# nellogrb/MultigridAnisotropicDiffusion

Hardware: AMD Instinct MI355X
Metric: Mvoxel-smooths/s (and V-cycles/s) at 512^3 fp32; achieved HBM GB/s vs peak (higher is better)
Workload: dtype f32

## Files before the change

### multigridanisotropicdiffusion_amd/build.py

```python
import os
import shutil
import subprocess
import sys

HERE = os.path.dirname(os.path.abspath(__file__))
CSRC = os.path.join(HERE, "csrc")
OUT = os.path.join(HERE, "libmad_hip.so")
SOURCES = ["mad_solver.hip"]
DEPS = ["../../include/mad.h", "../../include/mad_ved.h", "../../include/mad_ced.h",
        "../../include/mad_pm.h"]


def deps():
    return [f for f in os.listdir(CSRC) if f.endswith((".hip", ".hpp"))] + DEPS


def hipcc():
    for cand in (os.environ.get("HIPCC"), "/opt/rocm/bin/hipcc", shutil.which("hipcc")):
        if cand and os.path.exists(cand):
            return cand
    raise RuntimeError("hipcc not found")


def up_to_date():
    if not os.path.exists(OUT):
        return False
    t = os.path.getmtime(OUT)
    return all(os.path.getmtime(os.path.join(CSRC, d)) <= t for d in deps())


def build(force=False, verbose=True):
    if not force and up_to_date():
        return OUT
    cmd = [hipcc(), "--offload-arch=gfx950", "-O3", "-std=c++17", "-fPIC", "-shared",
           "-Wall", "-Wno-unused-function", "-o", OUT + ".tmp"]
    cmd += [os.path.join(CSRC, s) for s in SOURCES]
    cmd += ["-lrccl", "-lrocsolver", "-lrocblas"]
    if verbose:
        print(" ".join(cmd), flush=True)
    subprocess.check_call(cmd, cwd=HERE)
    os.replace(OUT + ".tmp", OUT)
    return OUT


if __name__ == "__main__":
    build(force="--force" in sys.argv)
```

### multigridanisotropicdiffusion_amd/csrc/mad_kernels.hpp

```cpp
#pragma once
#include <hip/hip_runtime.h>

#include <climits>
#include <type_traits>
#include <cstdint>

namespace mad {

enum { KISO = 1, KDIAG = 2, KFULL = 3 };

template <int DIM, int KIND>
struct CoefLayout {
  static constexpr int NA = (KIND == KISO) ? 1 : DIM;
  static constexpr int NG = DIM;
  static constexpr int NE = (KIND == KFULL) ? DIM * (DIM - 1) / 2 : 0;
  static constexpr int N = NA + NG + NE;
};

inline int coef_count(int dim, int kind) {
  int na = (kind == KISO) ? 1 : dim;
  int ne = (kind == KFULL) ? dim * (dim - 1) / 2 : 0;
  return na + dim + ne;
}

// ... 810 lines not shown
template <typename T, int DIM, int KIND>
__global__ void __launch_bounds__(256) residual_k(const T* __restrict__ u, const T* __restrict__ b,
                                                  T* __restrict__ r, const T* __restrict__ cf,
                                                  Geo g, Rat<T> rat, double* __restrict__ part) {
  const int k = (DIM == 3) ? (int)blockIdx.z : 0;
  const int j = blockIdx.y * blockDim.y + threadIdx.y;
  const int i = blockIdx.x * blockDim.x + threadIdx.x;
  double sq = 0.0;
  if (i < g.nx && j < g.ny) {
    const int64_t p = i + g.sy * j + g.sz * k;
    T D, S;
    stencil_terms<T, DIM, KIND>(u, cf, g, rat, i, j, k, p, D, S);
    const T rv = resid_value(b[p], D, u[p], S);
    r[p] = rv;
    sq = (double)rv * (double)rv;
  }
  if (part) {
    const double s = block_sum<256>(sq);
    if (threadIdx.x == 0 && threadIdx.y == 0)
      part[blockIdx.x + gridDim.x * (blockIdx.y + gridDim.y * blockIdx.z)] = s;
  }
}

template <typename T, int KIND, int TX, int TY, bool BREC = false, typename TE = T, typename TB = T>
__global__ void __launch_bounds__(TX * TY) resid3_k(const T* __restrict__ u, const TB* __restrict__ b,
                                                    T* __restrict__ r, const T* __restrict__ cf,
                                                    Geo g, Rat<T> rat, int zc, int ntx,
                                                    double* __restrict__ part,
                                                    TE* __restrict__ be = nullptr,
                                                    TE* __restrict__ xe = nullptr,
                                                    const TE* __restrict__ ue = nullptr,
                                                    T* __restrict__ uo = nullptr,
                                                    TE* __restrict__ bse = nullptr) {
  constexpr int NT = TX * TY;
  constexpr int RX = TX + 2, RY = TY + 2, PL = RX * RY;
  constexpr int UPT = (PL + NT - 1) / NT;
  constexpr int NCF = CoefLayout<3, KIND>::N;
  constexpr int RS = NCF + (BREC ? 1 : 0);
  constexpr uint32_t TS = sizeof(T);
  __shared__ T ring[4 * PL];
  const int tiles_per_plane = ntx * ((g.ny + TY - 1) / TY);
  const int chunk = blockIdx.x / tiles_per_plane;
  const int tile = blockIdx.x - chunk * tiles_per_plane;
  const int tyi = tile / ntx, txi = tile - (tile / ntx) * ntx;
  const int x0 = txi * TX, y0 = tyi * TY;
  const int tid = threadIdx.x;
  const int tx = tid % TX, ty = tid / TX;
// ... 5 lines not shown
  int u_dst[UPT];
  uint32_t u_src[UPT];
#pragma unroll
  for (int e = 0; e < UPT; ++e) {
    const int q = tid + e * NT;
    const int lj = q / RX, li = q - (q / RX) * RX;
    u_dst[e] = q < PL ? q : -1;
    u_src[e] = (uint32_t)(mirror(y0 - 1 + lj, ny) * sy + mirror(x0 - 1 + li, nx)) * TS;
  }
  const int i = x0 + tx, j = y0 + ty;
  const bool ok = i < nx && j < ny;
  const uint32_t rec_off = ok ? (uint32_t)(ty * sy + (tx & 1) * hx0 + (tx >> 1)) * (TS * RS) : 0u;
  const uint32_t pt_off = ok ? (uint32_t)(ty * sy + tx) * TS : 0u;
  const uint32_t pt_off_b = ok ? (uint32_t)(ty * sy + tx) * (uint32_t)sizeof(TB) : 0u;
  const int64_t rbase = (int64_t)y0 * sy + (x0 >> 1), pbase = (int64_t)y0 * sy + x0;
  const int il = (ty + 1) * RX + (tx + 1);
  constexpr int oyp = RX, oym = -RX;

  T up[UPT];
  T raw[RS];
  T bv = T(0);
  auto load_plane = [&](int m) {
    m = min(max(m, zlo), zhi - 1);
    const __amdgpu_buffer_rsrc_t rs = buf_rsrc(u + (int64_t)m * sz);
#pragma unroll
    for (int e = 0; e < UPT; ++e) up[e] = buf_load<T>(rs, u_src[e], 0u);
    if (ue) {
      const __amdgpu_buffer_rsrc_t re = buf_rsrc(ue + (int64_t)m * sz);
#pragma unroll
      for (int e = 0; e < UPT; ++e)
        up[e] = up[e] + (T)buf_load<TE>(re, (u_src[e] / TS) * (uint32_t)sizeof(TE), 0u);
    }
  };
  auto put_plane = [&](int m) {
    T* P = ring + (m & 3) * PL;
#pragma unroll
    for (int e = 0; e < UPT; ++e)
      if (e < UPT - 1 || u_dst[e] >= 0) P[u_dst[e]] = up[e];
  };
  auto load_pt = [&](int m) {
    m = min(max(m, 0), g.nz - 1);
    buf_load_rec<T, RS>(buf_rsrc(cf + ((int64_t)m * sz + rbase) * RS), rec_off, raw);
    if constexpr (!BREC) bv = (T)buf_load<TB>(buf_rsrc(b + (int64_t)m * sz + pbase), pt_off_b, 0u);
  };

  if (z0 - 1 >= zlo) {
// ... 627 lines not shown
            vz = fma(wy[bq], fma(wx[x][1], row[ix[x][1]], wx[x][0] * row[ix[x][0]]), vz);
          }
          v = fma(wz[c], vz, v);
        }
        out.v[x] = ADD ? xc[q].v[x] + v : v;
      }
      if (ok) *reinterpret_cast<V*>(fine + pxy + gf.sz * (int64_t)kk) = out;
    }
    __syncthreads();
#pragma unroll
    for (int q = 0; q < G; ++q) xc[q] = xn[q];
  }
}

template <typename T>
__global__ void __launch_bounds__(256) bsplit_k(const T* __restrict__ b, T* __restrict__ bs, Geo g, int p0) {
  const int k = p0 + (int)blockIdx.z;
  const int j = blockIdx.y * blockDim.y + threadIdx.y;
  const int i = blockIdx.x * blockDim.x + threadIdx.x;
  if (i >= g.nx || j >= g.ny) return;
  bs[cidx(g, i, j, k)] = b[i + g.sy * j + g.sz * (int64_t)k];
}

template <typename T>
__global__ void __launch_bounds__(256) brec_scatter_k(const T* __restrict__ b, T* __restrict__ cf,
                                                      Geo g, int ncf, int p0) {
  const int k = p0 + (int)blockIdx.z;
  const int j = blockIdx.y * blockDim.y + threadIdx.y;
  const int i = blockIdx.x * blockDim.x + threadIdx.x;
  if (i >= g.nx || j >= g.ny) return;
  cf[cidx(g, i, j, k) * g.rs + ncf] = b[i + g.sy * j + g.sz * (int64_t)k];
}

template <typename T>
__device__ __forceinline__ double coarse_row_dot(const double* __restrict__ a, const T* __restrict__ b,
                                                 int n, int lane) {
  double s = 0.0;
  for (int c = lane; c < n; c += 64) s += a[c] * (double)b[c];
  return wave_sum(s);
}

template <typename T>
__global__ void __launch_bounds__(256) coarse_solve_k(const double* __restrict__ inv,
                                                      const T* __restrict__ b, T* __restrict__ x,
                                                      int n) {
  const int row = blockIdx.x * 4 + (threadIdx.x >> 6);
// ... 356 lines not shown
```

### multigridanisotropicdiffusion_amd/csrc/mad_solver.hip

```cpp
#include <hip/hip_runtime.h>
#include <rocblas/rocblas.h>
#include <rocsolver/rocsolver.h>

#include <algorithm>
#include <chrono>
#include <cmath>
#include <cstdio>
#include <cstdlib>
#include <cstring>
#include <memory>
#include <mutex>
#include <stdexcept>
#include <string>
#include <thread>
#include <type_traits>
#include <vector>

#include "../../include/mad.h"
#include "mad_alloc.hpp"
#include "mad_coarse.hpp"
#include "mad_comm.hpp"
#include "mad_kernels.hpp"

using namespace mad;
// ... 852 lines not shown

  ZRange part_range(LevelData<T>& L, int tiles, const FusedCfg& fc, int part, int* flip,
                    uint32_t** sig) {
    const int nz = L.g.nz;
    ZRange zr = whole_range(nz, tiles, fc);
    *flip = (c_->d.gs_kernel == 4 && part == 0) ? 1 : 0;
    *sig = nullptr;
    if (part == 3 || part == 4) {
      REQUIRE(zr.nchunks >= 2 && zr.zc >= GHOST, MAD_ERR_UNSUPPORTED, "slab too thin for the single-launch sweep");
      *flip = 1;
      *sig = part == 3 ? L.sig : nullptr;
    } else if (part == 1) {
      zr = ZRange{0, boundary_planes(), nz - boundary_planes(), 2};
    } else if (part == 2) {
      const int ni = nz - 2 * boundary_planes();
      int chunks = std::max(1, std::min((fc.blocks + tiles - 1) / tiles, std::max(1, ni / 16)));
      const int zc = (ni + chunks - 1) / chunks;
      zr = ZRange{boundary_planes(), zc, zc, (ni + zc - 1) / zc};
    }
    return zr;
  }

  template <int KD, int TX, int TY, int NT>
  void launch_fused(LevelData<T>& L, const FusedCfg& fc, int part, bool zu = false) {
    const int ntx = (L.g.nx + TX - 1) / TX, nty = (L.g.ny + TY - 1) / TY;
    const int tiles = ntx * nty;
    int flip = 0;
    uint32_t* sig = nullptr;
    const ZRange zr = part_range(L, tiles, fc, part, &flip, &sig);
    const unsigned nb = (unsigned)(tiles * zr.nchunks);
    constexpr int NC = (KD == KFULL) ? 4 : 2;
    using FG = FusedGeom<NC, TX, TY>;
    constexpr size_t lds_u = sizeof(T) * FG::NP * FG::PLANE;
    REQUIRE(lds_u <= 160 * 1024, MAD_ERR_UNSUPPORTED,
            "fused GS tile needs " + std::to_string(lds_u) + " B of LDS (> 160 KiB)");
    constexpr size_t lds_bl = sizeof(T) * (FG::NP + NC) * FG::PLANE;
    constexpr bool bl_fits = lds_bl <= 160 * 1024;
    const bool bl = fused_b_lds(L);
    const size_t lds = bl ? lds_bl : lds_u;
    constexpr int MW = sizeof(T) == 8 ? 2 : 4;
    const PeerOut<T> po = part == 4 ? peer_out(L, buffer_index(L, L.t)) : PeerOut<T>{{nullptr, nullptr}, {nullptr, nullptr}};
    auto run = [&](auto kern) {
      {
        static std::mutex attr_mu;
        static std::vector<const void*> attr;
        std::lock_guard<std::mutex> lk(attr_mu);
        if (std::find(attr.begin(), attr.end(), (const void*)kern) == attr.end()) {
          HIP_CHECK(hipFuncSetAttribute((const void*)kern, hipFuncAttributeMaxDynamicSharedMemorySize,
                                        (int)lds));
          attr.push_back((const void*)kern);
        }
      }
      hipLaunchKernelGGL(kern, dim3(nb), dim3(NT), lds, c_->stream, L.x, L.t, L.bs ? L.bs : L.b, L.cf, L.g,
                         L.rat, zr.zc, ntx, nty, zr.zbase, zr.zstride, flip, sig, po);
    };
    if (part == 4) {
      if (L.brec)
        run(gs_fused3_k<T, KD, TX, TY, NT, MW, 2, true, true>);
      else if constexpr (bl_fits) {
        if (L.bs)
          run(gs_fused3_k<T, KD, TX, TY, NT, MW, 2, false, true, false, false, true>);
        else
          bl ? run(gs_fused3_k<T, KD, TX, TY, NT, MW, 2, false, true, true>)
             : run(gs_fused3_k<T, KD, TX, TY, NT, MW, 2, false, true>);
      } else
        run(gs_fused3_k<T, KD, TX, TY, NT, MW, 2, false, true>);
    } else if (L.brec) {
      run(gs_fused3_k<T, KD, TX, TY, NT, MW, 2, true>);
    } else if constexpr (bl_fits) {
      if (zu) {
        REQUIRE(part == 0, MAD_ERR_STATE, "zero-iterate sweep on a rank slab");
        if (L.bs)
          run(gs_fused3_k<T, KD, TX, TY, NT, MW, 2, false, false, false, true, true>);
        else
          bl ? run(gs_fused3_k<T, KD, TX, TY, NT, MW, 2, false, false, true, true>)
             : run(gs_fused3_k<T, KD, TX, TY, NT, MW, 2, false, false, false, true>);
      } else if (L.bs) {
        run(gs_fused3_k<T, KD, TX, TY, NT, MW, 2, false, false, false, false, true>);
// ... 4 lines not shown
    } else {
      REQUIRE(!zu, MAD_ERR_STATE, "zero-iterate sweep without its instance");
      run(gs_fused3_k<T, KD, TX, TY, NT, MW, 2>);
    }
  }

#ifndef MAD_FUSED_B_LDS
#define MAD_FUSED_B_LDS 1
#endif
  bool fused_b_lds(const LevelData<T>& L) const {
    return MAD_FUSED_B_LDS && sizeof(T) == 4 && !L.brec && !L.bs && &L == &lv_[0];
  }

#ifndef MAD_FUSED_F32_TY
#define MAD_FUSED_F32_TY 32
#endif
  void fused_shape(const LevelData<T>& L, int* tiles, int* nchunks) const {
    const FusedCfg fc = fused_cfg();
    const int tx = 64, ty = (c_->kind == KFULL && sizeof(T) == 4) ? MAD_FUSED_F32_TY : 16;
    *tiles = ((L.g.nx + tx - 1) / tx) * ((L.g.ny + ty - 1) / ty);
    *nchunks = whole_range(L.g.nz, *tiles, fc).nchunks;
  }

  void launch_fused_part(LevelData<T>& L, int part, bool zu = false) {
    const FusedCfg fc = fused_cfg();
    if (c_->kind == KFULL) {
      if constexpr (sizeof(T) == 4)
        launch_fused<KFULL, 64, MAD_FUSED_F32_TY, MAD_FUSED_F32_TY * 32>(L, fc, part, zu);
      else
        launch_fused<KFULL, 64, 16, 512>(L, fc, part, zu);
    } else if (c_->kind == KDIAG) {
      launch_fused<KDIAG, 64, 16, 1024>(L, fc, part, zu);
    } else {
      launch_fused<KISO, 64, 16, 1024>(L, fc, part, zu);
    }
    HIP_CHECK(hipGetLastError());
  }

  std::string smooth_kernel(int l) override {
    (void)l;
    const char* tn = sizeof(T) == 4 ? "float" : "double";
    const int dim = c_->dim, kind = c_->kind;
    char buf[160];
    if (c_->d.smoother == MAD_WEIGHTED_JACOBI) {
      const LevelData<T>& L = lv_[l];
      if (dim == 3 && L.g.nx >= 16 && L.g.ny >= 16)
        std::snprintf(buf, sizeof buf, "wj3_k<%s, %d, 64, 16, %s>", tn, kind, L.brec ? "true" : "false");
      else
        std::snprintf(buf, sizeof buf, "wj_k<%s, %d, %d>", tn, dim, kind);
    } else if (c_->d.smoother == MAD_GAUSS_SEIDEL_LEX) {
      std::snprintf(buf, sizeof buf, "gs_lex_plane_k<%s, %d, %d>", tn, dim, kind);
    } else if (!use_fused(l)) {
      std::snprintf(buf, sizeof buf, "gs_color_k<%s, %d, %d>", tn, dim, kind);
      if (lv_[l].peer) return std::string(buf) + " [rank slab: peer halo, edge planes pushed after the last colour pass]";
    } else {
      const int tx = 64, ty = (kind == KFULL && sizeof(T) == 4) ? MAD_FUSED_F32_TY : 16;
      const int nt = (kind == KFULL && sizeof(T) == 8) ? 512 : (kind == KFULL ? MAD_FUSED_F32_TY * 32 : 1024);
// ... 75 lines not shown
      std::swap(L.x, L.t);
      std::swap(L.alloc[0], L.alloc[3]);
      L.x_halo_ok = true;
      L.x_peer_pending = true;
      return 0.f;
    }
    const bool overlap = sweep_overlap(l);
    int tiles = 0, nchunks = 0;
    if (overlap) fused_shape(L, &tiles, &nchunks);
    if (overlap && L.sig && nchunks >= 2) {
      launch_fused_part(L, 3);
      wait_all_pending();
      const uint32_t target = ++L.sig_epoch * (uint32_t)tiles;
      if (L.g.zlo_ghost)
        HIP_CHECK(hipStreamWaitValue32(c_->comm_stream, L.sig, target, hipStreamWaitValueGte, 0xFFFFFFFFu));
      if (L.g.zhi_ghost)
        HIP_CHECK(hipStreamWaitValue32(c_->comm_stream, L.sig + 1, target, hipStreamWaitValueGte,
                                       0xFFFFFFFFu));
      c_->comm.exchange_planes(L.t, L.g.sz, L.g.nz, GHOST, L.g.zlo_ghost, L.g.zhi_ghost, sizeof(T),
                               std::is_same<T, double>::value, c_->comm_stream);
      HIP_CHECK(hipEventRecord(L.ev_halo, c_->comm_stream));
    } else if (!overlap) {
      const bool zu = (zero_x0_ && &L == &lv_[0]) || L.x_zero_lazy;
      zero_x0_ = false;
      L.x_zero_lazy = false;
      launch_fused_part(L, 0, zu);
    } else {
      launch_fused_part(L, 1);
      wait_all_pending();
      HIP_CHECK(hipEventRecord(L.ev_bnd, c_->stream));
      HIP_CHECK(hipStreamWaitEvent(c_->comm_stream, L.ev_bnd, 0));
      c_->comm.exchange_planes(L.t, L.g.sz, L.g.nz, GHOST, L.g.zlo_ghost, L.g.zhi_ghost, sizeof(T),
                               std::is_same<T, double>::value, c_->comm_stream);
      HIP_CHECK(hipEventRecord(L.ev_halo, c_->comm_stream));
      launch_fused_part(L, 2);
    }
    if (e1) HIP_CHECK(hipEventRecord(e1, c_->stream));
    std::swap(L.x, L.t);
    std::swap(L.alloc[0], L.alloc[3]);
    if (overlap) {
      L.x_halo_ok = true;
      L.x_halo_pending = true;
    } else {
      L.x_halo_ok = false;
    }
    return 0.f;
  }

  void prep_wj(int l) {
// ... 98 lines not shown
  }

  double finish_norm2(int64_t nparts, bool global) {
    hipLaunchKernelGGL(reduce_final_k, dim3(1), dim3(256), 0, c_->stream, part_, nparts, scal_);
    HIP_CHECK(hipGetLastError());
    if (global && c_->comm.active()) {
      wait_all_pending();
      c_->comm.allreduce_sum_f64(scal_, 1, c_->stream);
    }
    HIP_CHECK(hipMemcpyAsync(hscal_, scal_, sizeof(double), hipMemcpyDeviceToHost, c_->stream));
    HIP_CHECK(hipStreamSynchronize(c_->stream));
    return hscal_[0];
  }

  double residual(int l, bool want_norm) override { return residual_impl(l, want_norm, true); }

  bool refine_emitted_ = false;
  bool refine_emitted_bs_ = false;
  bool refine_fold_ok() const {
    const LevelData<T>& L = lv_[0];
    return c_->dim == 3 && L.g.nx >= 16 && L.g.ny >= 16 && !c_->geom[0].distributed;
  }
  bool zero_x0_ = false;
  bool lazy_zero_ok(int l) const {
#ifdef MAD_NO_LAZY_ZERO
    return false;
#else
    const auto& d = c_->d;
    return sizeof(T) == 4 && l >= 1 && l < c_->nlev - 1 && !c_->comm.active() && !d.verbose &&
           d.iterations_per_grid >= 1 && use_fused(l) && d.gs_kernel != 4 && !lv_[l].brec &&
           c_->dim == 3;
#endif
  }
  bool zero_sweep_ok() const {
#ifdef MAD_NO_ZERO_SWEEP
    return false;
#else
    const auto& d = c_->d;
    return sizeof(T) == 4 && refine_fold_ok() && !c_->comm.active() && d.cycle == MAD_VCYCLE &&
           !d.verbose && d.iterations_per_grid >= 1 && c_->nlev > 1 && use_fused(0) && d.gs_kernel != 4 &&
           !lv_[0].brec;
#endif
  }
  double residual64(bool fold = false) {
    LevelData<T>& L = lv_[0];
    if (fold && !refine_fold_ok()) {
      hipLaunchKernelGGL((add_conv_k<T>), dim3(flat_blocks(L.g.N)), dim3(256), 0, c_->stream, u64_, L.x, L.g.N);
      HIP_CHECK(hipGetLastError());
      fold = false;
    }
    if (c_->comm.active() && c_->geom[0].distributed) {
      wait_all_pending();
      c_->comm.exchange_planes(u64_, L.g.sz, L.g.nz, 1, L.g.zlo_ghost, L.g.zhi_ghost, sizeof(double),
                               true, c_->stream);
    }
    Geo g = L.g;
    g.rs = ncoef_;
    int64_t nparts = 0;
    if (c_->dim == 3 && g.nx >= 16 && g.ny >= 16) {
      constexpr int TX = 64, TY = 16;
      const int ntx = (g.nx + TX - 1) / TX, nty = (g.ny + TY - 1) / TY;
      int chunks = std::max(1, std::min((1024 + ntx * nty - 1) / (ntx * nty), g.nz / 8));
      const int zc = (g.nz + chunks - 1) / chunks;
      chunks = (g.nz + zc - 1) / zc;
      nparts = (int64_t)ntx * nty * chunks;
      REQUIRE(nparts <= part_cap_, MAD_ERR_UNSUPPORTED, "residual partials buffer too small");
      T* const bse = (L.bs && !c_->geom[0].distributed) ? L.bs : nullptr;
      refine_emitted_bs_ = bse != nullptr;
      auto go = [&](auto K) {
        constexpr int KD = decltype(K)::value;
        auto launch = [&](auto bptr) {
          using TB = std::remove_const_t<std::remove_pointer_t<decltype(bptr)>>;
          if (fold)
            hipLaunchKernelGGL((resid3_k<double, KD, TX, TY, false, T, TB>), dim3((unsigned)nparts),
                               dim3(TX * TY), 0, c_->stream, u64_, bptr, (double*)nullptr, cf64_, g, rat64_, zc,
                               ntx, part_, L.b, (T*)nullptr, (const T*)L.x, r64_, bse);
          else
            hipLaunchKernelGGL((resid3_k<double, KD, TX, TY, false, T, TB>), dim3((unsigned)nparts),
                               dim3(TX * TY), 0, c_->stream, u64_, bptr, (double*)nullptr, cf64_, g, rat64_, zc,
                               ntx, part_, L.b, L.x, (const T*)nullptr, (double*)nullptr, bse);
        };
#ifdef MAD_NO_B32_RHS
        launch((const double*)b64_);
#else
        if (b32_exact_)
          launch((const float*)b32_);
        else
          launch((const double*)b64_);
#endif
      };
      refine_emitted_ = true;
      if (c_->kind == KFULL) go(std::integral_constant<int, KFULL>{});
      else if (c_->kind == KDIAG) go(std::integral_constant<int, KDIAG>{});
      else go(std::integral_constant<int, KISO>{});
      if (fold) {
        std::swap(u64_, r64_);
        if (!zero_sweep_ok())
          hipLaunchKernelGGL((fill_k<T>), dim3(flat_blocks(L.g.N)), dim3(256), 0, c_->stream, L.x, L.g.N, T(0));
      }
    } else {
      dim3 gr = grid_for(g.nx, g.ny, g.nz, BLK);
      nparts = (int64_t)gr.x * gr.y * gr.z;
      REQUIRE(nparts <= part_cap_, MAD_ERR_UNSUPPORTED, "residual partials buffer too small");
      dispatch(c_->dim, c_->kind, [&](auto D, auto K) {
        hipLaunchKernelGGL((residual_k<double, D.value, K.value>), gr, BLK, 0, c_->stream, u64_, b64_,
                           r64_, cf64_, g, rat64_, part_);
      });
      refine_emitted_ = refine_emitted_bs_ = false;
    }
    HIP_CHECK(hipGetLastError());
    return std::sqrt(finish_norm2(nparts, c_->geom[0].distributed));
  }

  double norm64(const double* a) {
    const int64_t n = lv_[0].g.N;
    unsigned nb = flat_blocks(n, 2048);
    hipLaunchKernelGGL((sumsq_k<double>), dim3(nb), dim3(256), 0, c_->stream, a, n, part_);
    HIP_CHECK(hipGetLastError());
// ... 279 lines not shown
      lv_[0].x_halo_ok = false;
    if (!lv_[0].brec && !lv_[0].b_halo_ok) {
      halo(0, lv_[0].b, GHOST);
      lv_[0].b_halo_ok = true;
    }
    wait_all_pending();
    for (size_t l = 1; l < lv_.size(); ++l) {
      lv_[l].x_halo_ok = false;
      lv_[l].b_halo_ok = lv_[l].brec_ok = false;
    }
  }

  void vcycle_fast() {
    const bool ranks = c_->comm.active();
    if (c_->d.verbose || c_->bench_trace() || vgraph_failed_ || (ranks && !vgraph_ranks_ok()) ||
        (ranks && vcycles_eager_ < 1)) {
      if (ranks) ++vcycles_eager_;
      vcycle_rec(0);
      return;
    }
    sync_brec(0);
    sync_bsplit(0);
    if (ranks) ranks_graph_entry();
    const bool zu = zero_x0_;
    if (vgraph_) {
      bool same = vgraph_ptrs_.size() == lv_.size() && vgraph_zu_ == zu;
      for (size_t l = 0; same && l < lv_.size(); ++l)
        same = vgraph_ptrs_[l].first == lv_[l].x && vgraph_ptrs_[l].second == lv_[l].t &&
               vgraph_seq_[l] == (lv_[l].peer_seq & 1);
      if (!same) {
        HIP_CHECK(hipStreamSynchronize(c_->stream));
        (void)hipGraphExecDestroy(vgraph_);
        vgraph_ = nullptr;
      }
    }
    if (!vgraph_) {
      struct Snap {
        T* x;
        T* t;
        T* a0;
        T* a3;
        bool bh;
        int seq;
      };
      auto snap = [&] {
        std::vector<Snap> v;
        for (auto& L : lv_) v.push_back({L.x, L.t, L.alloc[0], L.alloc[3], L.b_halo_ok, L.peer_seq});
        return v;
      };
      auto restore = [&](const std::vector<Snap>& v) {
        for (size_t l = 0; l < lv_.size(); ++l) {
          lv_[l].x = v[l].x;
          lv_[l].t = v[l].t;
          lv_[l].alloc[0] = v[l].a0;
          lv_[l].alloc[3] = v[l].a3;
          lv_[l].b_halo_ok = v[l].bh;
          lv_[l].peer_seq = v[l].seq;
        }
      };
// ... 5 lines not shown
      try {
        vcycle_rec(0);
        if (ranks) {
          wait_all_pending();
          peer_resolve_all();
        }
      } catch (...) {
        (void)hipStreamEndCapture(c_->stream, &gph);
        if (gph) (void)hipGraphDestroy(gph);
        gph = nullptr;
        restore(before);
        if (!ranks) throw;
        captured = false;
      }
      if (captured && hipStreamEndCapture(c_->stream, &gph) != hipSuccess) {
        gph = nullptr;
        captured = false;
      }
      const std::vector<Snap> after = snap();
      bool same = captured;
      for (size_t l = 0; same && l < before.size(); ++l)
        same = before[l].x == after[l].x && before[l].t == after[l].t &&
               ((before[l].seq ^ after[l].seq) & 1) == 0;
      vgraph_exit_flags_ = halo_flags();
      restore(before);
      if (ranks) {
        for (size_t l = 0; l < lv_.size(); ++l) {
          lv_[l].x_halo_ok = flags_before[l].x_ok;
          lv_[l].b_halo_ok = flags_before[l].b_ok;
          lv_[l].brec_ok = flags_before[l].brec_ok;
          lv_[l].x_halo_pending = false;
        }
      }
      if (same && hipGraphInstantiate(&vgraph_, gph, nullptr, nullptr, 0) != hipSuccess) {
        vgraph_ = nullptr;
        same = false;
      }
      if (gph) (void)hipGraphDestroy(gph);
      zero_x0_ = zu;
      if (!same) {
        (void)hipGetLastError();
        vgraph_failed_ = true;
        vcycle_rec(0);
        return;
      }
      vgraph_zu_ = zu;
      zero_x0_ = false;
      vgraph_ptrs_.clear();
      vgraph_seq_.clear();
      for (auto& L : lv_) {
        vgraph_ptrs_.emplace_back(L.x, L.t);
        vgraph_seq_.push_back(L.peer_seq & 1);
      }
    }
    HIP_CHECK(hipGraphLaunch(vgraph_, c_->stream));
    zero_x0_ = false;
    if (ranks) c_->comm.graph_launched(c_->stream);
    if (ranks) {
      for (size_t l = 0; l < lv_.size(); ++l) {
        lv_[l].x_halo_ok = vgraph_exit_flags_[l].x_ok;
        lv_[l].b_halo_ok = vgraph_exit_flags_[l].b_ok;
        lv_[l].brec_ok = vgraph_exit_flags_[l].brec_ok;
        lv_[l].x_halo_pending = false;
      }
    } else {
      for (size_t l = 1; l < lv_.size(); ++l) lv_[l].b_halo_ok = lv_[l].brec_ok = false;
    }
  }

  void vcycle() override { vcycle_fast(); }

  void fmg() override { fmg_rec(0); }

  void per_sweep_line(int l, int it, const char* what, bool bench) {
    if (!c_->d.verbose) {
      const double rn = residual(l, true);
      c_->trace_push(c_->trace_rhs > 0.0 ? rn / c_->trace_rhs : rn);
      return;
    }
    const double rel = verbose_line(l, it, what);
    if (bench) {
      const double rn = rel * norm(l, MAD_B);
      c_->trace_push(c_->trace_rhs > 0.0 ? rn / c_->trace_rhs : rn);
    }
  }
// ... 29 lines not shown
    }
    if (refine_) {
      convert_to(src, in_dtype, b64_, N, c_->stream);
      b32_exact_ = in_dtype == MAD_U8 || in_dtype == MAD_I8 || in_dtype == MAD_U16 || in_dtype == MAD_I16 ||
                   in_dtype == MAD_F32;
      if (b32_exact_) {
        hipLaunchKernelGGL((convert_k<double, float>), dim3(nb), dim3(256), 0, c_->stream, b64_, b32_, N);
        HIP_CHECK(hipGetLastError());
      }
    } else {
      convert_in(src, in_dtype, L0.b, N);
      L0.b_halo_ok = L0.brec_ok = false;
    }
    auto to_fp32_rhs = [&](const double* a) {
      hipLaunchKernelGGL((convert_k<double, T>), dim3(nb), dim3(256), 0, c_->stream, a, L0.b, N);
      HIP_CHECK(hipGetLastError());
      L0.b_halo_ok = L0.brec_ok = false;
    };
    auto x_to_u64 = [&] {
      hipLaunchKernelGGL((convert_k<T, double>), dim3(nb), dim3(256), 0, c_->stream, L0.x, u64_, N);
      HIP_CHECK(hipGetLastError());
    };
    auto rhs_norm = [&] { return refine_ ? norm64(b64_) : norm(0, MAD_B); };
    Event e0, e1;
    HIP_CHECK(hipEventRecord(e0, c_->stream));
    c_->step_cycles.clear();
    c_->step_relres.clear();
    c_->trace.clear();
    const bool bt = c_->bench_trace();
    FlagScope tracing(c_->trace_active);
    c_->trace_t0 = std::chrono::steady_clock::now();
    bool stalled_any = false;
    unsigned total = 0;
    double relres = 0.0;
    for (unsigned step = 0; step < d.number_of_steps; ++step) {
      if (d.verbose && d.number_of_steps > 1 && c_->comm.rank() == 0)
        std::printf("\n------------ Time step n. %u / %u------------\n", step + 1, d.number_of_steps);
#ifdef MAD_NO_REFINE_FP32_PHASE
      const bool fp32_phase = false;
#else
      const bool fp32_phase = refine_ && d.cycle != MAD_SMOOTHER && d.max_cycles >= 2;
#endif
      if (bt) {
        c_->trace_t0 = std::chrono::steady_clock::now();
        c_->trace_step = step;
        c_->trace_rhs = rhs_norm();
      }
      if (refine_ && (d.cycle == MAD_FMG || fp32_phase)) to_fp32_rhs(b64_);
      if (d.cycle == MAD_FMG) {
        if (d.verbose && c_->comm.rank() == 0) std::printf("|--- Full Multigrid Cycle ---|\n");
        fmg_rec(0);
        if (refine_ && !fp32_phase) x_to_u64();
      } else if (!refine_ || fp32_phase) {
        HIP_CHECK(hipMemcpyAsync(L0.x, L0.b, sizeof(T) * N, hipMemcpyDeviceToDevice, c_->stream));
        x_changed(0);
      } else {
        HIP_CHECK(hipMemcpyAsync(u64_, b64_, sizeof(double) * N, hipMemcpyDeviceToDevice, c_->stream));
      }
      const double rhsNorm = rhs_norm();
      REQUIRE(std::isfinite(rhsNorm), MAD_ERR_NUMERIC,
              "non-finite right-hand side norm (NaN/Inf in the input image)");
      unsigned it = 0;
      std::vector<double> hist;
      const unsigned window = (d.cycle == MAD_SMOOTHER) ? 50 : 5;
      bool stalled = false;
      auto rel = [&](double resNorm) {
        REQUIRE(std::isfinite(resNorm), MAD_ERR_NUMERIC,
                "non-finite residual norm (NaN/Inf in the tensor or the iterate)");
        return (rhsNorm > 0.0) ? resNorm / rhsNorm : resNorm;
      };
      auto cycle = [&](bool zero_x0) {
        if (d.cycle == MAD_SMOOTHER) {
          smooth(0, 1);
          return;
        }
        if (d.verbose && c_->comm.rank() == 0) std::printf("\n|--- VCycle n. %u ---|\n", it + 1);
        FlagScope zu(zero_x0_, zero_x0);
        vcycle_fast();
      };
      auto record = [&](double resNorm) {
        relres = rel(resNorm);
        if (d.verbose && d.cycle == MAD_SMOOTHER && c_->comm.rank() == 0)
          std::printf("Smoother iteration n. %u: relative residual = %g\n", it + 1, relres);
        ++it;
        hist.push_back(relres);
        if (!bt || d.cycle == MAD_SMOOTHER) {
          c_->trace_step = step;
          c_->trace_push(relres);
        }
      };
      if (fp32_phase) {
        do {
          cycle(false);
          record(residual_impl(0, true, false));
          if (hist.size() >= 2 && relres > MAD_REFINE_FP32_MIN_RATE * hist[hist.size() - 2]) break;
        } while (relres > std::max(d.tolerance, MAD_REFINE_SWITCH_RELRES) && it + 1 < d.max_cycles);
        x_to_u64();
      }
      auto patch_trace = [&] {
        if (!c_->trace.empty()) c_->trace.back().relres = relres;
      };
      if (refine_) {
        relres = rel(residual64());
        if (fp32_phase) {
          hist.back() = relres;
          patch_trace();
        }
      }
      if (!fp32_phase || (relres > d.tolerance && it < d.max_cycles)) do {
        if (!refine_) {
          cycle(false);
          record(residual_impl(0, true, false));
        } else {
          if (refine_emitted_) {
            L0.b_halo_ok = false;
            L0.brec_ok = refine_emitted_bs_;
            x_changed(0);
          } else {
            to_fp32_rhs(r64_);
            fill(0, MAD_X, 0.0);
          }
          cycle(refine_emitted_ && zero_sweep_ok());
          record(residual64(true));
          if (bt && d.cycle != MAD_SMOOTHER) patch_trace();
        }
        stalled = d.stall_guard && stalled_at(hist, window, d.tolerance);
      } while (relres > d.tolerance && it < d.max_cycles && !stalled);
      stalled_any |= stalled;
      total += it;
      c_->step_cycles.push_back(it);
      c_->step_relres.push_back(relres);
      if (refine_) {
        HIP_CHECK(hipMemcpyAsync(b64_, u64_, sizeof(double) * N, hipMemcpyDeviceToDevice, c_->stream));
        b32_exact_ = false;
      } else {
        HIP_CHECK(hipMemcpyAsync(L0.b, L0.x, sizeof(T) * N, hipMemcpyDeviceToDevice, c_->stream));
        L0.b_halo_ok = L0.brec_ok = false;
      }
    }
    HIP_CHECK(hipEventRecord(e1, c_->stream));
    if (refine_ && refine_emitted_ && zero_sweep_ok()) fill(0, MAD_X, 0.0);
    void* dst = out;
    if (!dev_io) dst = scratch_bytes(N * dtype_size(out_dtype));
    if (refine_) convert_from(u64_, dst, out_dtype, N, c_->stream);
    else convert_out(L0.x, dst, out_dtype, N);
    if (!dev_io)
      HIP_CHECK(hipMemcpyAsync(out, dst, N * dtype_size(out_dtype), hipMemcpyDeviceToHost,
                               c_->stream));
    HIP_CHECK(hipStreamSynchronize(c_->stream));
    peer_check();
    if (st) {
      std::memset(st, 0, sizeof(*st));
      st->steps = d.number_of_steps;
      st->total_cycles = total;
      st->last_cycles = c_->step_cycles.empty() ? 0 : c_->step_cycles.back();
      st->stalled = stalled_any ? 1 : 0;
      st->last_relres = relres;
      st->setup_ms = c_->setup_ms;
      st->solve_ms = elapsed(e0, e1);
      st->num_levels = (uint32_t)c_->nlev;
      st->tensor_kind = c_->kind;
      st->colors = c_->ncolors;
    }
  }

  void bench_smooth(int l, unsigned n, double* total_ms, double* kern_ms,
                    unsigned* launches) override {
// ... 58 lines not shown
    Event a, z;
    HIP_CHECK(hipEventRecord(a, c_->stream));
    for (unsigned s = 0; s < n; ++s) vcycle_fast();
    HIP_CHECK(hipEventRecord(z, c_->stream));
    HIP_CHECK(hipEventSynchronize(z));
    *total_ms = elapsed(a, z);
  }

 private:
  mad_ctx* c_ = nullptr;
  std::vector<LevelData<T>> lv_;
  bool refine_ = false;
  double* r64alloc_[3] = {nullptr, nullptr, nullptr};
  double* u64_ = nullptr;
  double* b64_ = nullptr;
  float* b32alloc_ = nullptr;
  float* b32_ = nullptr;
  bool b32_exact_ = false;
  double* r64_ = nullptr;
  double* cf64_alloc_ = nullptr;
  double* cf64_ = nullptr;
  Rat<double> rat64_{};
  int64_t part_cap_ = 0;
  hipGraphExec_t vgraph_ = nullptr;
  bool vgraph_zu_ = false;
  std::vector<std::pair<T*, T*>> vgraph_ptrs_;
  std::vector<int> vgraph_seq_;
  bool vgraph_failed_ = false;
  uint64_t peer_timeout_ticks_ = 0;
  int peer_fallbacks_ = 0;
  std::vector<HaloFlags> vgraph_exit_flags_;
  int vcycles_eager_ = 0;
  int ncoef_ = 0;
  double* part_ = nullptr;
  double* scal_ = nullptr;
  double* hscal_ = nullptr;
  double* inv_ = nullptr;
  CoarseBlocks cblk_;
  void* scratch_ = nullptr;
  size_t scratch_cap_ = 0;
  T* gathered_ = nullptr;
  T* full_x_ = nullptr;
  int64_t gathered_cap_ = 0;
  T* cslab_ = nullptr;
  int64_t cslab_cap_ = 0;

  void release() {
    if (c_ && c_->comm_stream) (void)hipStreamSynchronize(c_->comm_stream);
    if (c_ && c_->comm.mode() != Comm::LOCAL) {
      try {
        for (size_t l = 0; l < lv_.size(); ++l)
          if (lv_[l].x_peer_pending) peer_resolve((int)l);
      } catch (...) {
      }
    }
    if (c_ && c_->stream) (void)hipStreamSynchronize(c_->stream);
    if (vgraph_) (void)hipGraphExecDestroy(vgraph_);
    vgraph_ = nullptr;
    vgraph_ptrs_.clear();
    vgraph_seq_.clear();
    vgraph_failed_ = false;
    vcycles_eager_ = 0;
    for (auto& L : lv_) {
      if (L.ev_bnd) (void)hipEventDestroy(L.ev_bnd);
      if (L.ev_halo) (void)hipEventDestroy(L.ev_halo);
      if (L.sig) (void)hipFree(L.sig);
      Comm::close_window(L.win_lo, L.win_ipc);
      Comm::close_window(L.win_hi, L.win_ipc);
      if (L.win) (void)hipFree(L.win);
      for (auto& a : L.alloc)
        if (a) (void)hipFree(a);
      if (L.cf_alloc) (void)hipFree(L.cf_alloc);
      if (L.bs_alloc) (void)hipFree(L.bs_alloc);
    }
    lv_.clear();
    for (auto& a : r64alloc_)
      if (a) (void)hipFree(a), a = nullptr;
    if (cf64_alloc_) (void)hipFree(cf64_alloc_);
    cf64_alloc_ = nullptr;
    u64_ = b64_ = r64_ = cf64_ = nullptr;
    if (b32alloc_) (void)hipFree(b32alloc_);
    b32alloc_ = b32_ = nullptr;
    b32_exact_ = false;
// ... 1126 lines not shown
```

Before: 118,300.

## Fuse per-step RHS conversion, split and norm; drop initial copies and fp64 swaps

Adds a step_rhs_k kernel that converts the right-hand side, writes the split/coloured copy and computes its norm in one pass, replacing separate conversion, bsplit and norm launches. The first smoothing sweep can read its initial iterate directly from b instead of copying b into x, which needs a third cached V-cycle graph variant. The fp64 residual at the precision switch reads the fp32 iterate directly, skipping x_to_u64, and the per-step b64/u64 copy becomes a pointer swap. This removes several full-volume memory passes per time step, at the cost of more graph variants and state flags, and a build variant with the fusion disabled.

```diff
diff --git a/multigridanisotropicdiffusion_amd/build.py b/multigridanisotropicdiffusion_amd/build.py
--- a/multigridanisotropicdiffusion_amd/build.py
+++ b/multigridanisotropicdiffusion_amd/build.py
@@ -6,6 +6,8 @@
 HERE = os.path.dirname(os.path.abspath(__file__))
 CSRC = os.path.join(HERE, "csrc")
 OUT = os.path.join(HERE, "libmad_hip.so")
+VARIANTS = [(OUT, []),
+            (os.path.join(HERE, "libmad_hip_nostepfusion.so"), ["-DMAD_NO_STEP_FUSION"])]
 SOURCES = ["mad_solver.hip"]
 DEPS = ["../../include/mad.h", "../../include/mad_ved.h", "../../include/mad_ced.h",
         "../../include/mad_pm.h"]
@@ -23,23 +25,32 @@
 
 
 def up_to_date():
-    if not os.path.exists(OUT):
-        return False
-    t = os.path.getmtime(OUT)
-    return all(os.path.getmtime(os.path.join(CSRC, d)) <= t for d in deps())
+    for out, _ in VARIANTS:
+        if not os.path.exists(out):
+            return False
+        t = os.path.getmtime(out)
+        if not all(os.path.getmtime(os.path.join(CSRC, d)) <= t for d in deps()):
+            return False
+    return True
 
 
 def build(force=False, verbose=True):
     if not force and up_to_date():
         return OUT
-    cmd = [hipcc(), "--offload-arch=gfx950", "-O3", "-std=c++17", "-fPIC", "-shared",
-           "-Wall", "-Wno-unused-function", "-o", OUT + ".tmp"]
-    cmd += [os.path.join(CSRC, s) for s in SOURCES]
-    cmd += ["-lrccl", "-lrocsolver", "-lrocblas"]
-    if verbose:
-        print(" ".join(cmd), flush=True)
-    subprocess.check_call(cmd, cwd=HERE)
-    os.replace(OUT + ".tmp", OUT)
+    procs = []
+    for out, flags in VARIANTS:
+        cmd = [hipcc(), "--offload-arch=gfx950", "-O3", "-std=c++17", "-fPIC", "-shared",
+               "-Wall", "-Wno-unused-function"] + flags + ["-o", out + ".tmp"]
+        cmd += [os.path.join(CSRC, s) for s in SOURCES]
+        cmd += ["-lrccl", "-lrocsolver", "-lrocblas"]
+        if verbose:
+            print(" ".join(cmd), flush=True)
+        procs.append((out, cmd, subprocess.Popen(cmd, cwd=HERE)))
+    failed = [(cmd, p.returncode) for out, cmd, p in procs if p.wait() != 0]
+    if failed:
+        raise subprocess.CalledProcessError(failed[0][1], failed[0][0])
+    for out, _, _ in procs:
+        os.replace(out + ".tmp", out)
     return OUT
 
 
diff --git a/multigridanisotropicdiffusion_amd/csrc/mad_kernels.hpp b/multigridanisotropicdiffusion_amd/csrc/mad_kernels.hpp
--- a/multigridanisotropicdiffusion_amd/csrc/mad_kernels.hpp
+++ b/multigridanisotropicdiffusion_amd/csrc/mad_kernels.hpp
@@ -856,7 +856,8 @@
   }
 }
 
-template <typename T, int KIND, int TX, int TY, bool BREC = false, typename TE = T, typename TB = T>
+template <typename T, int KIND, int TX, int TY, bool BREC = false, typename TE = T, typename TB = T,
+          bool UE = false>
 __global__ void __launch_bounds__(TX * TY) resid3_k(const T* __restrict__ u, const TB* __restrict__ b,
                                                     T* __restrict__ r, const T* __restrict__ cf,
                                                     Geo g, Rat<T> rat, int zc, int ntx,
@@ -908,6 +909,12 @@
   T bv = T(0);
   auto load_plane = [&](int m) {
     m = min(max(m, zlo), zhi - 1);
+    if constexpr (UE) {
+      const __amdgpu_buffer_rsrc_t re = buf_rsrc(ue + (int64_t)m * sz);
+#pragma unroll
+      for (int e = 0; e < UPT; ++e) up[e] = (T)buf_load<TE>(re, (u_src[e] / TS) * (uint32_t)sizeof(TE), 0u);
+      return;
+    }
     const __amdgpu_buffer_rsrc_t rs = buf_rsrc(u + (int64_t)m * sz);
 #pragma unroll
     for (int e = 0; e < UPT; ++e) up[e] = buf_load<T>(rs, u_src[e], 0u);
@@ -1581,6 +1588,43 @@
   bs[cidx(g, i, j, k)] = b[i + g.sy * j + g.sz * (int64_t)k];
 }
 
+template <typename S, typename T>
+__global__ void __launch_bounds__(256) step_rhs_k(const S* __restrict__ src, T* __restrict__ b,
+                                                  T* __restrict__ bs, Geo g, int64_t n,
+                                                  double* __restrict__ part) {
+  double s = 0.0;
+  const int64_t stride = (int64_t)gridDim.x * blockDim.x;
+  const int row = (int)g.sy, rows = (int)(g.sz / g.sy);
+  int64_t q = blockIdx.x * (int64_t)blockDim.x + threadIdx.x;
+  int k = (int)(q / g.sz);
+  int j = (int)((q - k * g.sz) / row);
+  int i = (int)(q - k * g.sz - (int64_t)j * row);
+  const int dk = (int)(stride / g.sz);
+  const int dj = (int)((stride - dk * g.sz) / row);
+  const int di = (int)(stride - dk * g.sz - (int64_t)dj * row);
+  for (; q < n; q += stride) {
+    const S raw = src[q];
+    const double v = (double)raw;
+    s += v * v;
+    const T bv = (T)raw;
+    if (b) b[q] = bv;
+    if (bs) bs[cidx(g, i, j, k)] = bv;
+    i += di;
+    j += dj;
+    k += dk;
+    if (i >= row) {
+      i -= row;
+      ++j;
+    }
+    if (j >= rows) {
+      j -= rows;
+      ++k;
+    }
+  }
+  s = block_sum<256>(s);
+  if (threadIdx.x == 0) part[blockIdx.x] = s;
+}
+
 template <typename T>
 __global__ void __launch_bounds__(256) brec_scatter_k(const T* __restrict__ b, T* __restrict__ cf,
                                                       Geo g, int ncf, int p0) {
diff --git a/multigridanisotropicdiffusion_amd/csrc/mad_solver.hip b/multigridanisotropicdiffusion_amd/csrc/mad_solver.hip
--- a/multigridanisotropicdiffusion_amd/csrc/mad_solver.hip
+++ b/multigridanisotropicdiffusion_amd/csrc/mad_solver.hip
@@ -898,7 +898,7 @@
   }
 
   template <int KD, int TX, int TY, int NT>
-  void launch_fused(LevelData<T>& L, const FusedCfg& fc, int part, bool zu = false) {
+  void launch_fused(LevelData<T>& L, const FusedCfg& fc, int part, bool zu = false, const T* uin = nullptr) {
     const int ntx = (L.g.nx + TX - 1) / TX, nty = (L.g.ny + TY - 1) / TY;
     const int tiles = ntx * nty;
     int flip = 0;
@@ -927,9 +927,11 @@
           attr.push_back((const void*)kern);
         }
       }
-      hipLaunchKernelGGL(kern, dim3(nb), dim3(NT), lds, c_->stream, L.x, L.t, L.bs ? L.bs : L.b, L.cf, L.g,
+      hipLaunchKernelGGL(kern, dim3(nb), dim3(NT), lds, c_->stream, uin ? uin : (const T*)L.x, L.t,
+                         L.bs ? L.bs : L.b, L.cf, L.g,
                          L.rat, zr.zc, ntx, nty, zr.zbase, zr.zstride, flip, sig, po);
     };
+    REQUIRE(!uin || (part == 0 && !zu), MAD_ERR_STATE, "input override on a rank slab or a zero-iterate sweep");
     if (part == 4) {
       if (L.brec)
         run(gs_fused3_k<T, KD, TX, TY, NT, MW, 2, true, true>);
@@ -980,17 +982,17 @@
     *nchunks = whole_range(L.g.nz, *tiles, fc).nchunks;
   }
 
-  void launch_fused_part(LevelData<T>& L, int part, bool zu = false) {
+  void launch_fused_part(LevelData<T>& L, int part, bool zu = false, const T* uin = nullptr) {
     const FusedCfg fc = fused_cfg();
     if (c_->kind == KFULL) {
       if constexpr (sizeof(T) == 4)
-        launch_fused<KFULL, 64, MAD_FUSED_F32_TY, MAD_FUSED_F32_TY * 32>(L, fc, part, zu);
+        launch_fused<KFULL, 64, MAD_FUSED_F32_TY, MAD_FUSED_F32_TY * 32>(L, fc, part, zu, uin);
       else
-        launch_fused<KFULL, 64, 16, 512>(L, fc, part, zu);
+        launch_fused<KFULL, 64, 16, 512>(L, fc, part, zu, uin);
     } else if (c_->kind == KDIAG) {
-      launch_fused<KDIAG, 64, 16, 1024>(L, fc, part, zu);
+      launch_fused<KDIAG, 64, 16, 1024>(L, fc, part, zu, uin);
     } else {
-      launch_fused<KISO, 64, 16, 1024>(L, fc, part, zu);
+      launch_fused<KISO, 64, 16, 1024>(L, fc, part, zu, uin);
     }
     HIP_CHECK(hipGetLastError());
   }
@@ -1112,9 +1114,10 @@
       HIP_CHECK(hipEventRecord(L.ev_halo, c_->comm_stream));
     } else if (!overlap) {
       const bool zu = (zero_x0_ && &L == &lv_[0]) || L.x_zero_lazy;
-      zero_x0_ = false;
+      const T* uin = (b_x0_ && &L == &lv_[0] && !zu) ? L.b : nullptr;
+      zero_x0_ = b_x0_ = false;
       L.x_zero_lazy = false;
-      launch_fused_part(L, 0, zu);
+      launch_fused_part(L, 0, zu, uin);
     } else {
       launch_fused_part(L, 1);
       wait_all_pending();
@@ -1259,6 +1262,15 @@
     return c_->dim == 3 && L.g.nx >= 16 && L.g.ny >= 16 && !c_->geom[0].distributed;
   }
   bool zero_x0_ = false;
+  bool b_x0_ = false;
+  bool lean_steps() const {
+#ifdef MAD_NO_STEP_FUSION
+    return false;
+#else
+    return sizeof(T) == 4 && c_->dim == 3 && !c_->comm.active() && !c_->geom[0].distributed &&
+           !c_->d.verbose && !c_->bench_trace() && lv_[0].g.sz <= (int64_t)INT32_MAX;
+#endif
+  }
   bool lazy_zero_ok(int l) const {
 #ifdef MAD_NO_LAZY_ZERO
     return false;
@@ -1279,8 +1291,9 @@
            !lv_[0].brec;
 #endif
   }
-  double residual64(bool fold = false) {
+  double residual64(bool fold = false, bool from_x = false) {
     LevelData<T>& L = lv_[0];
+    REQUIRE(!from_x || (!fold && refine_fold_ok()), MAD_ERR_STATE, "fp32 iterate in the per-point fp64 residual");
     if (fold && !refine_fold_ok()) {
       hipLaunchKernelGGL((add_conv_k<T>), dim3(flat_blocks(L.g.N)), dim3(256), 0, c_->stream, u64_, L.x, L.g.N);
       HIP_CHECK(hipGetLastError());
@@ -1308,7 +1321,11 @@
         constexpr int KD = decltype(K)::value;
         auto launch = [&](auto bptr) {
           using TB = std::remove_const_t<std::remove_pointer_t<decltype(bptr)>>;
-          if (fold)
+          if (from_x)
+            hipLaunchKernelGGL((resid3_k<double, KD, TX, TY, false, T, TB, true>), dim3((unsigned)nparts),
+                               dim3(TX * TY), 0, c_->stream, (const double*)nullptr, bptr, (double*)nullptr, cf64_,
+                               g, rat64_, zc, ntx, part_, L.b, (T*)nullptr, (const T*)L.x, r64_, bse);
+          else if (fold)
             hipLaunchKernelGGL((resid3_k<double, KD, TX, TY, false, T, TB>), dim3((unsigned)nparts),
                                dim3(TX * TY), 0, c_->stream, u64_, bptr, (double*)nullptr, cf64_, g, rat64_, zc,
                                ntx, part_, L.b, (T*)nullptr, (const T*)L.x, r64_, bse);
@@ -1330,7 +1347,7 @@
       if (c_->kind == KFULL) go(std::integral_constant<int, KFULL>{});
       else if (c_->kind == KDIAG) go(std::integral_constant<int, KDIAG>{});
       else go(std::integral_constant<int, KISO>{});
-      if (fold) {
+      if (fold || from_x) {
         std::swap(u64_, r64_);
         if (!zero_sweep_ok())
           hipLaunchKernelGGL((fill_k<T>), dim3(flat_blocks(L.g.N)), dim3(256), 0, c_->stream, L.x, L.g.N, T(0));
@@ -1656,19 +1673,20 @@
     sync_brec(0);
     sync_bsplit(0);
     if (ranks) ranks_graph_entry();
-    const bool zu = zero_x0_;
-    if (vgraph_) {
-      bool same = vgraph_ptrs_.size() == lv_.size() && vgraph_zu_ == zu;
+    const bool zu = zero_x0_, bu = b_x0_;
+    VGraph& G = vgraphs_[zu ? 1 : (bu ? 2 : 0)];
+    if (G.exec) {
+      bool same = G.ptrs.size() == lv_.size();
       for (size_t l = 0; same && l < lv_.size(); ++l)
-        same = vgraph_ptrs_[l].first == lv_[l].x && vgraph_ptrs_[l].second == lv_[l].t &&
-               vgraph_seq_[l] == (lv_[l].peer_seq & 1);
+        same = G.ptrs[l].first == lv_[l].x && G.ptrs[l].second == lv_[l].t &&
+               G.seq[l] == (lv_[l].peer_seq & 1);
       if (!same) {
         HIP_CHECK(hipStreamSynchronize(c_->stream));
-        (void)hipGraphExecDestroy(vgraph_);
-        vgraph_ = nullptr;
-      }
-    }
-    if (!vgraph_) {
+        (void)hipGraphExecDestroy(G.exec);
+        G.exec = nullptr;
+      }
+    }
+    if (!G.exec) {
       struct Snap {
         T* x;
         T* t;
@@ -1720,7 +1738,7 @@
       for (size_t l = 0; same && l < before.size(); ++l)
         same = before[l].x == after[l].x && before[l].t == after[l].t &&
                ((before[l].seq ^ after[l].seq) & 1) == 0;
-      vgraph_exit_flags_ = halo_flags();
+      G.exit_flags = halo_flags();
       restore(before);
       if (ranks) {
         for (size_t l = 0; l < lv_.size(); ++l) {
@@ -1730,35 +1748,35 @@
           lv_[l].x_halo_pending = false;
         }
       }
-      if (same && hipGraphInstantiate(&vgraph_, gph, nullptr, nullptr, 0) != hipSuccess) {
-        vgraph_ = nullptr;
+      if (same && hipGraphInstantiate(&G.exec, gph, nullptr, nullptr, 0) != hipSuccess) {
+        G.exec = nullptr;
         same = false;
       }
       if (gph) (void)hipGraphDestroy(gph);
       zero_x0_ = zu;
+      b_x0_ = bu;
       if (!same) {
         (void)hipGetLastError();
         vgraph_failed_ = true;
         vcycle_rec(0);
         return;
       }
-      vgraph_zu_ = zu;
-      zero_x0_ = false;
-      vgraph_ptrs_.clear();
-      vgraph_seq_.clear();
+      zero_x0_ = b_x0_ = false;
+      G.ptrs.clear();
+      G.seq.clear();
       for (auto& L : lv_) {
-        vgraph_ptrs_.emplace_back(L.x, L.t);
-        vgraph_seq_.push_back(L.peer_seq & 1);
-      }
-    }
-    HIP_CHECK(hipGraphLaunch(vgraph_, c_->stream));
-    zero_x0_ = false;
+        G.ptrs.emplace_back(L.x, L.t);
+        G.seq.push_back(L.peer_seq & 1);
+      }
+    }
+    HIP_CHECK(hipGraphLaunch(G.exec, c_->stream));
+    zero_x0_ = b_x0_ = false;
     if (ranks) c_->comm.graph_launched(c_->stream);
     if (ranks) {
       for (size_t l = 0; l < lv_.size(); ++l) {
-        lv_[l].x_halo_ok = vgraph_exit_flags_[l].x_ok;
-        lv_[l].b_halo_ok = vgraph_exit_flags_[l].b_ok;
-        lv_[l].brec_ok = vgraph_exit_flags_[l].brec_ok;
+        lv_[l].x_halo_ok = G.exit_flags[l].x_ok;
+        lv_[l].b_halo_ok = G.exit_flags[l].b_ok;
+        lv_[l].brec_ok = G.exit_flags[l].brec_ok;
         lv_[l].x_halo_pending = false;
       }
     } else {
@@ -1834,6 +1852,24 @@
       HIP_CHECK(hipGetLastError());
     };
     auto rhs_norm = [&] { return refine_ ? norm64(b64_) : norm(0, MAD_B); };
+    auto rhs_prologue = [&] {
+      const unsigned nbn = flat_blocks(N, 2048);
+      if (!refine_)
+        hipLaunchKernelGGL((step_rhs_k<T, T>), dim3(nbn), dim3(256), 0, c_->stream, (const T*)L0.b, (T*)nullptr,
+                           L0.bs, L0.g, N, part_);
+      else if (b32_exact_)
+        hipLaunchKernelGGL((step_rhs_k<float, T>), dim3(nbn), dim3(256), 0, c_->stream, (const float*)b32_, L0.b,
+                           L0.bs, L0.g, N, part_);
+      else
+        hipLaunchKernelGGL((step_rhs_k<double, T>), dim3(nbn), dim3(256), 0, c_->stream, (const double*)b64_,
+                           L0.b, L0.bs, L0.g, N, part_);
+      HIP_CHECK(hipGetLastError());
+      L0.b_halo_ok = false;
+      L0.brec_ok = L0.bs != nullptr;
+      return std::sqrt(finish_norm2(nbn, false));
+    };
+    const bool lean = lean_steps();
+    const double* sol64 = u64_;
     Event e0, e1;
     HIP_CHECK(hipEventRecord(e0, c_->stream));
     c_->step_cycles.clear();
@@ -1858,18 +1894,26 @@
         c_->trace_step = step;
         c_->trace_rhs = rhs_norm();
       }
-      if (refine_ && (d.cycle == MAD_FMG || fp32_phase)) to_fp32_rhs(b64_);
+      const bool vc = lean && d.cycle == MAD_VCYCLE;
+      const bool prologue = vc && (refine_ ? fp32_phase : (L0.bs != nullptr && !L0.brec));
+      const bool b_first = vc && (!refine_ || fp32_phase) && zero_sweep_ok();
+      const bool switch_from_x = lean && fp32_phase && refine_fold_ok();
+      double prologue_norm = 0.0;
+      if (prologue)
+        prologue_norm = rhs_prologue();
+      else if (refine_ && (d.cycle == MAD_FMG || fp32_phase))
+        to_fp32_rhs(b64_);
       if (d.cycle == MAD_FMG) {
         if (d.verbose && c_->comm.rank() == 0) std::printf("|--- Full Multigrid Cycle ---|\n");
         fmg_rec(0);
         if (refine_ && !fp32_phase) x_to_u64();
       } else if (!refine_ || fp32_phase) {
-        HIP_CHECK(hipMemcpyAsync(L0.x, L0.b, sizeof(T) * N, hipMemcpyDeviceToDevice, c_->stream));
+        if (!b_first) HIP_CHECK(hipMemcpyAsync(L0.x, L0.b, sizeof(T) * N, hipMemcpyDeviceToDevice, c_->stream));
         x_changed(0);
       } else {
         HIP_CHECK(hipMemcpyAsync(u64_, b64_, sizeof(double) * N, hipMemcpyDeviceToDevice, c_->stream));
       }
-      const double rhsNorm = rhs_norm();
+      const double rhsNorm = prologue ? prologue_norm : rhs_norm();
       REQUIRE(std::isfinite(rhsNorm), MAD_ERR_NUMERIC,
               "non-finite right-hand side norm (NaN/Inf in the input image)");
       unsigned it = 0;
@@ -1888,6 +1932,7 @@
         }
         if (d.verbose && c_->comm.rank() == 0) std::printf("\n|--- VCycle n. %u ---|\n", it + 1);
         FlagScope zu(zero_x0_, zero_x0);
+        FlagScope bu(b_x0_, b_first && it == 0 && !zero_x0);
         vcycle_fast();
       };
       auto record = [&](double resNorm) {
@@ -1907,13 +1952,13 @@
           record(residual_impl(0, true, false));
           if (hist.size() >= 2 && relres > MAD_REFINE_FP32_MIN_RATE * hist[hist.size() - 2]) break;
         } while (relres > std::max(d.tolerance, MAD_REFINE_SWITCH_RELRES) && it + 1 < d.max_cycles);
-        x_to_u64();
+        if (!switch_from_x) x_to_u64();
       }
       auto patch_trace = [&] {
         if (!c_->trace.empty()) c_->trace.back().relres = relres;
       };
       if (refine_) {
-        relres = rel(residual64());
+        relres = rel(residual64(false, switch_from_x));
         if (fp32_phase) {
           hist.back() = relres;
           patch_trace();
@@ -1943,7 +1988,13 @@
       c_->step_cycles.push_back(it);
       c_->step_relres.push_back(relres);
       if (refine_) {
-        HIP_CHECK(hipMemcpyAsync(b64_, u64_, sizeof(double) * N, hipMemcpyDeviceToDevice, c_->stream));
+        if (lean) {
+          std::swap(b64_, u64_);
+          sol64 = b64_;
+        } else {
+          HIP_CHECK(hipMemcpyAsync(b64_, u64_, sizeof(double) * N, hipMemcpyDeviceToDevice, c_->stream));
+          sol64 = u64_;
+        }
         b32_exact_ = false;
       } else {
         HIP_CHECK(hipMemcpyAsync(L0.b, L0.x, sizeof(T) * N, hipMemcpyDeviceToDevice, c_->stream));
@@ -1954,7 +2005,7 @@
     if (refine_ && refine_emitted_ && zero_sweep_ok()) fill(0, MAD_X, 0.0);
     void* dst = out;
     if (!dev_io) dst = scratch_bytes(N * dtype_size(out_dtype));
-    if (refine_) convert_from(u64_, dst, out_dtype, N, c_->stream);
+    if (refine_) convert_from(sol64, dst, out_dtype, N, c_->stream);
     else convert_out(L0.x, dst, out_dtype, N);
     if (!dev_io)
       HIP_CHECK(hipMemcpyAsync(out, dst, N * dtype_size(out_dtype), hipMemcpyDeviceToHost,
@@ -2059,14 +2110,16 @@
   double* cf64_ = nullptr;
   Rat<double> rat64_{};
   int64_t part_cap_ = 0;
-  hipGraphExec_t vgraph_ = nullptr;
-  bool vgraph_zu_ = false;
-  std::vector<std::pair<T*, T*>> vgraph_ptrs_;
-  std::vector<int> vgraph_seq_;
+  struct VGraph {
+    hipGraphExec_t exec = nullptr;
+    std::vector<std::pair<T*, T*>> ptrs;
+    std::vector<int> seq;
+    std::vector<HaloFlags> exit_flags;
+  };
+  VGraph vgraphs_[3];
   bool vgraph_failed_ = false;
   uint64_t peer_timeout_ticks_ = 0;
   int peer_fallbacks_ = 0;
-  std::vector<HaloFlags> vgraph_exit_flags_;
   int vcycles_eager_ = 0;
   int ncoef_ = 0;
   double* part_ = nullptr;
@@ -2092,10 +2145,10 @@
       }
     }
     if (c_ && c_->stream) (void)hipStreamSynchronize(c_->stream);
-    if (vgraph_) (void)hipGraphExecDestroy(vgraph_);
-    vgraph_ = nullptr;
-    vgraph_ptrs_.clear();
-    vgraph_seq_.clear();
+    for (auto& G : vgraphs_) {
+      if (G.exec) (void)hipGraphExecDestroy(G.exec);
+      G = VGraph{};
+    }
     vgraph_failed_ = false;
     vcycles_eager_ = 0;
     for (auto& L : lv_) {
```

Measured after the change: 118,400, median of 2. No clear change (+0.1%).
